# rainerzufalldererste/hypersonic-rANS

Hardware: AMD Instinct MI355X
Metric: decode MiB/s (bit-exact) on 100 MB stream (higher is better)
Workload: dtype u32 state / u16 word / u8 symbol (integer)

## Files before the change

hypersonic_rans_amd/csrc/kernels_common.h:

```cpp
#ifndef HSRANS_KERNELS_COMMON_H
#define HSRANS_KERNELS_COMMON_H

namespace hsrans
{


typedef uint32_t u32x4 __attribute__((ext_vector_type(4)));

constexpr uint32_t kRingSlots = 4;
constexpr uint32_t kChunkBytes = 512;
constexpr uint32_t kRingBytes = kRingSlots * kChunkBytes;
constexpr uint32_t kWaveRingBytes = kRingBytes + 256;
constexpr uint32_t kFastRingBytes = kRingBytes + kChunkBytes;
constexpr uint32_t kConsume = 1u << 15;
#ifndef HSRANS_HAVE_STAMPS
#define HSRANS_HAVE_STAMPS 0
#endif
#define HSRANS_STAMPS(kp) (HSRANS_HAVE_STAMPS && (kp).stamps != nullptr)
constexpr uint32_t kSingleMirror = 256;

constexpr int kModePack = 0;
constexpr int kModePackM1 = 1;
constexpr int kModeTwoLevel = 2;
constexpr int kModePack64 = 3;

constexpr int kModeRank = 4;
constexpr int kModeSpill = 5;

__host__ __device__ constexpr uint32_t table_bytes_for(int mode, uint32_t bits)
{
  return mode == kModeSpill ? 0u
         : mode == kModeTwoLevel ? (1u << bits) + 1024
         : mode == kModePack64 ? 8u << bits
         : mode == kModeRank ? (1u << bits) + 2048u
                               : 4u << bits;
}

__host__ __device__ constexpr bool fast_ring_mode(int mode) { return mode == kModePack64 || mode == kModeRank; }
__host__ __device__ constexpr bool table_first_mode(int mode) { return mode == kModeRank; }

__device__ __forceinline__ uint32_t lds_address(const void *p)
{
  return (uint32_t)(uintptr_t)(const __attribute__((address_space(3))) uint8_t *)p;
}
__device__ __forceinline__ uint32_t uni(uint32_t v) { return __builtin_amdgcn_readfirstlane(v); }
__device__ __forceinline__ uint64_t uni64(uint64_t v)
{
  return (uint64_t)uni((uint32_t)v) | ((uint64_t)uni((uint32_t)(v >> 32)) << 32);
}

#ifndef HSRANS_STORE_POLICY
#define HSRANS_STORE_POLICY " nt"
#endif
#ifndef HSRANS_STORE_POLICY_DIRECT
#define HSRANS_STORE_POLICY_DIRECT " sc0 sc1"
#endif
#define HSRANS_STORE_U32(ptr, v) asm volatile("global_store_dword %0, %1, off" HSRANS_STORE_POLICY : : "v"(ptr), "v"(v) : "memory")
#define HSRANS_STORE_U32_SADDR(base, voff, v) asm volatile("global_store_dword %0, %1, %2" HSRANS_STORE_POLICY : : "v"(voff), "v"(v), "s"(base) : "memory")
template <bool WT>
__device__ __forceinline__ void store_u32(uint8_t *ptr, uint32_t v)
{
  if (WT)
    asm volatile("global_store_dword %0, %1, off" HSRANS_STORE_POLICY_DIRECT : : "v"(ptr), "v"(v) : "memory");
  else
    asm volatile("global_store_dword %0, %1, off" HSRANS_STORE_POLICY : : "v"(ptr), "v"(v) : "memory");
}
template <bool WT>
__device__ __forceinline__ void store_u32_saddr(uint8_t *base, uint32_t voff, uint32_t v)
{
  if (WT)
    asm volatile("global_store_dword %0, %1, %2" HSRANS_STORE_POLICY_DIRECT : : "v"(voff), "v"(v), "s"(base) : "memory");
  else
    asm volatile("global_store_dword %0, %1, %2" HSRANS_STORE_POLICY : : "v"(voff), "v"(v), "s"(base) : "memory");
}

template <bool WT>
__device__ __forceinline__ void store_u8(uint8_t *ptr, uint32_t v)
{
  if (WT)
    asm volatile("global_store_byte %0, %1, off sc0 sc1" : : "v"(ptr), "v"(v) : "memory");
  else
    *ptr = (uint8_t)v;
}
template <bool WT>
__device__ __forceinline__ void store_u128(u32x4 *ptr, u32x4 v)
{
  if (WT)
    asm volatile("global_store_dwordx4 %0, %1, off sc0 sc1" : : "v"(ptr), "v"(v) : "memory");
  else
    *ptr = v;
}

__device__ __forceinline__ uint64_t groups_of(uint32_t S, uint64_t bytes) { return S == 64 ? bytes >> 6 : S == 32 ? bytes >> 5 : bytes / S; }
struct Recip
{
  uint32_t d, inv;
};
__host__ __device__ __forceinline__ Recip recip_of(uint32_t d)
{
  Recip r;
  r.d = d ? d : 1;
  r.inv = 0xFFFFFFFFu / r.d;
  return r;
}
__device__ __forceinline__ uint32_t share_of(uint32_t a, uint32_t n, const Recip &r)
{
  const uint64_t wide = (uint64_t)a * n;
  if (wide >> 32)
    return (uint32_t)(wide / r.d);
  const uint32_t v = (uint32_t)wide;
  uint32_t q = __umulhi(v, r.inv);
  if (v - q * r.d >= r.d)
    q++;
  return q;
}

#define HSRANS_HIST_IN_RANGE(c, off) ((off) >= (c).stream_lo && (off) <= (c).stream_len && (c).stream_len - (off) >= 512)

__device__ __forceinline__ uint32_t lane_to_byte(uint32_t j) { return (j & 0x23u) | ((j & 0x04u) << 2) | ((j & 0x18u) >> 1); }

struct WaveCtx
{
  const uint8_t *stream;
  uint64_t stream_len;
  uint64_t stream_lo;
  uint8_t *out;
  uint64_t out_cap;
  uint32_t *status;
  uint32_t bits, S, lane;
  uint32_t v_mask, v_bits;
  uint8_t *rings;
  uint8_t *table;
  uint8_t *table_b;
  const uint2 *gtable;
  uint16_t *scratch_cnt;
  uint16_t *scratch_cum;
};

#define HSRANS_STREAM_LOAD_FLAGS ""
struct StreamWin
{
  u32x4 rs;
  uint64_t base;
};

struct Ring
{
  uint32_t voff0;
  uint32_t k;
  uint32_t cur;
  uint32_t lds;
  uint32_t clog;
  uint32_t mirror_lanes;
  uint32_t vm, seq1, seq2, seq3;
  uint32_t st1, st2;
#if HSRANS_HAVE_STAMPS
  uint32_t diag_wait = 0, diag_store = 0;
#endif
};

__device__ __forceinline__ void ring_bind(Ring &r, const uint8_t *lds_ring, uint32_t clog = 9, bool whole_chunk_mirror = false)
{
  r.lds = uni(lds_address(lds_ring));
  r.clog = clog;
  r.mirror_lanes = whole_chunk_mirror ? (clog == 9 ? 0xFFFFFFFFu : 0xFFFFu) : clog == 9 ? 0xFFu : 0xFu;
}
__device__ __forceinline__ uint32_t ring_bytes(const Ring &r) { return kRingSlots << r.clog; }

__device__ __forceinline__ void ring_request(const StreamWin &sw, const Ring &r, const WaveCtx &c, uint32_t chunk, bool with_mirror = true)
{
  const uint32_t voff = r.voff0 + (chunk << r.clog) + c.lane * 16;
  const uint32_t slot = chunk & (kRingSlots - 1);
  const uint32_t dst = uni(r.lds + (slot << r.clog));
  const uint32_t lanes = r.clog == 9 ? 0xFFFFFFFFu : 0xFFFFu;
  asm volatile("s_nop 4\n\ts_mov_b32 m0, %1\n\ts_mov_b64 exec, %3\n\tbuffer_load_dwordx4 %0, %2, 0 offen" HSRANS_STREAM_LOAD_FLAGS " lds\n\ts_mov_b64 exec, -1"
               :
               : "v"(voff), "s"(dst), "s"(sw.rs), "s"((uint64_t)lanes)
               : "memory");
  if (slot == 0 && with_mirror)
    asm volatile("s_mov_b32 m0, %1\n\ts_mov_b64 exec, %3\n\tbuffer_load_dwordx4 %0, %2, 0 offen" HSRANS_STREAM_LOAD_FLAGS " lds\n\ts_mov_b64 exec, -1"
                 :
                 : "v"(voff), "s"(uni(r.lds + ring_bytes(r))), "s"(sw.rs), "s"((uint64_t)r.mirror_lanes)
                 : "memory");
}

__device__ __forceinline__ void ring_request_mirror0(const StreamWin &sw, const Ring &r, const WaveCtx &c)
{
  const uint32_t voff = r.voff0 + c.lane * 16;
  asm volatile("s_nop 4\n\ts_mov_b32 m0, %1\n\ts_mov_b64 exec, %3\n\tbuffer_load_dwordx4 %0, %2, 0 offen" HSRANS_STREAM_LOAD_FLAGS " lds\n\ts_mov_b64 exec, -1"
               :
               : "v"(voff), "s"(uni(r.lds + ring_bytes(r))), "s"(sw.rs), "s"((uint64_t)r.mirror_lanes)
               : "memory");
}

__device__ __forceinline__ void win_open(StreamWin &sw, const WaveCtx &c, uint64_t pos, uint64_t limit)
{
  pos = uni64(pos);
  limit = uni64(limit);
  if (limit > c.stream_len)
    limit = c.stream_len;
  const uint64_t a0 = pos & ~(uint64_t)15;
  const uint64_t left = a0 < limit && a0 >= c.stream_lo ? (limit - a0 + 15) & ~(uint64_t)15 : 0;
  const uint64_t addr = (uint64_t)(uintptr_t)c.stream + a0;
  sw.rs.x = uni((uint32_t)addr);
  sw.rs.y = uni((uint32_t)(addr >> 32) & 0xFFFF);
  sw.rs.z = uni((uint32_t)(left > 0xFFFFFFFFull ? 0xFFFFFFFFull : left));
  sw.rs.w = 0x00020000;
  sw.base = a0;
}

#ifndef HSRANS_RING_AHEAD
#define HSRANS_RING_AHEAD 3
#endif
static_assert(HSRANS_RING_AHEAD == 2 || HSRANS_RING_AHEAD == 3, "the ring has 4 slots: the cursor's chunk + 2 or 3 requested ones");

__device__ __forceinline__ void ring_begin(const StreamWin &sw, Ring &r, const WaveCtx &c, uint64_t pos, bool issue = true, bool later = false)
{
  pos = uni64(pos);
  const uint32_t rel = (uint32_t)(pos - sw.base);
  r.voff0 = rel & ~15u;
  r.cur = (rel - r.voff0) >> 1;
  r.k = 0;
  r.st1 = r.st2 = 0;
  r.vm = 0;
  if (issue)
  {
    ring_request(sw, r, c, 0, !later);
    ring_request(sw, r, c, 1);
  }
  r.vm += 3;
  r.seq1 = r.vm;
  if (issue && !later)
    ring_request(sw, r, c, 2);
  r.seq2 = ++r.vm;
  if (HSRANS_RING_AHEAD == 3)
  {
    if (issue && !later)
      ring_request(sw, r, c, 3);
    r.vm++;
  }
  r.seq3 = r.vm;
}
__device__ __forceinline__ void ring_begin_rest(const StreamWin &sw, Ring &r, const WaveCtx &c)
{
  ring_request_mirror0(sw, r, c);
  ring_request(sw, r, c, 2);
  if (HSRANS_RING_AHEAD == 3)
    ring_request(sw, r, c, 3);
}

__device__ __forceinline__ void ring_ready()
{
  if (HSRANS_RING_AHEAD == 3)
    asm volatile("s_waitcnt vmcnt(2)" ::: "memory");
  else
    asm volatile("s_waitcnt vmcnt(1)" ::: "memory");
}
__device__ __forceinline__ void ring_ready(uint32_t &x)
{
  if (HSRANS_RING_AHEAD == 3)
    asm volatile("s_waitcnt vmcnt(2)" : "+v"(x)::"memory");
  else
    asm volatile("s_waitcnt vmcnt(1)" : "+v"(x)::"memory");
}
__device__ __forceinline__ void ring_ready(uint32_t &xa, uint32_t &xb)
{
  if (HSRANS_RING_AHEAD == 3)
    asm volatile("s_waitcnt vmcnt(2)" : "+v"(xa), "+v"(xb)::"memory");
  else
    asm volatile("s_waitcnt vmcnt(1)" : "+v"(xa), "+v"(xb)::"memory");
}

__device__ __forceinline__ void ring_init(StreamWin &sw, Ring &r, const WaveCtx &c, uint64_t pos, uint32_t &x)
{
  win_open(sw, c, pos, c.stream_len);
  ring_begin(sw, r, c, pos);
  ring_ready(x);
}

__device__ __forceinline__ void ring_advance(const StreamWin &sw, Ring &r, const WaveCtx &c)
{
  if ((r.cur >> (r.clog - 1)) > r.k)
  {
    r.k++;
    ring_request(sw, r, c, r.k + HSRANS_RING_AHEAD);
    r.vm += ((r.k + HSRANS_RING_AHEAD) & (kRingSlots - 1)) == 0 ? 2 : 1;
    r.seq1 = r.seq2;
    r.seq2 = r.seq3;
    r.seq3 = r.vm;
    if (HSRANS_RING_AHEAD == 2)
      r.seq2 = r.vm;
    asm volatile("s_waitcnt vmcnt(2)" ::: "memory");
  }
}

__device__ __forceinline__ void wait_vm_at_most(uint32_t n)
{
  if (n >= 8)
    asm volatile("s_waitcnt vmcnt(8)" ::: "memory");
  else if (n >= 6)
    asm volatile("s_waitcnt vmcnt(6)" ::: "memory");
  else if (n >= 4)
    asm volatile("s_waitcnt vmcnt(4)" ::: "memory");
  else if (n >= 2)
    asm volatile("s_waitcnt vmcnt(2)" ::: "memory");
  else if (n == 1)
    asm volatile("s_waitcnt vmcnt(1)" ::: "memory");
  else
    asm volatile("s_waitcnt vmcnt(0)" ::: "memory");
}

__device__ __forceinline__ void ring_advance_exact(const StreamWin &sw, Ring &r, const WaveCtx &c)
{
  if ((r.cur >> (r.clog - 1)) > r.k)
  {
    r.k++;
    ring_request(sw, r, c, r.k + HSRANS_RING_AHEAD);
    r.vm += ((r.k + HSRANS_RING_AHEAD) & (kRingSlots - 1)) == 0 ? 2 : 1;
    r.seq1 = r.seq2;
    r.seq2 = r.seq3;
    r.seq3 = r.vm;
    if (HSRANS_RING_AHEAD == 2)
      r.seq2 = r.vm;
    wait_vm_at_most(r.vm - r.seq1);
  }
}

__device__ __forceinline__ uint64_t ring_pos(const StreamWin &sw, const Ring &r) { return sw.base + r.voff0 + (uint64_t)r.cur * 2; }

__host__ __device__ constexpr bool pack64_marks(uint32_t total, uint32_t nthreads)
{
  return (nthreads & (nthreads - 1)) == 0 && nthreads >= 64 && total >= 1024 && total / (nthreads < total / 4 ? nthreads : total / 4) <= 8;
}
template <int CTRL, int ROW_MASK>
__device__ __forceinline__ uint32_t max_dpp(uint32_t v)
{
  const uint32_t o = (uint32_t)__builtin_amdgcn_update_dpp(0, (int)v, CTRL, ROW_MASK, 0xF, true);
  return v > o ? v : o;
}
__device__ __forceinline__ uint32_t wave_scan_max(uint32_t v)
{
  v = max_dpp<0x111, 0xF>(v);
  v = max_dpp<0x112, 0xF>(v);
  v = max_dpp<0x114, 0xF>(v);
  v = max_dpp<0x118, 0xF>(v);
  v = max_dpp<0x142, 0xA>(v);
  v = max_dpp<0x143, 0xC>(v);
  return v;
}
__device__ __forceinline__ void pack64_zero_marks(uint2 *tab, uint32_t total, uint32_t tid, uint32_t nthreads)
{
  for (uint32_t q = tid; q < total / 4; q += nthreads)
    ((uint32_t *)tab)[q] = 0;
}
__device__ __forceinline__ void pack64_mark4(uint2 *tab, uint32_t total, uint32_t s0, uint32_t excl, uint32_t c0, uint32_t c1, uint32_t c2, uint32_t c3)
{
  uint8_t *mk = (uint8_t *)tab;
  const uint32_t u0 = excl, u1 = u0 + c0, u2 = u1 + c1, u3 = u2 + c2;
  if (c0 != 0 && u0 < total)
    mk[u0] = (uint8_t)s0;
  if (c1 != 0 && u1 < total)
    mk[u1] = (uint8_t)(s0 + 1);
  if (c2 != 0 && u2 < total)
    mk[u2] = (uint8_t)(s0 + 2);
  if (c3 != 0 && u3 < total)
    mk[u3] = (uint8_t)(s0 + 3);
}
template <typename SYNC>
__device__ __forceinline__ void pack64_from_marks(uint2 *tab, const uint16_t *cnt, const uint16_t *cum, uint32_t total, uint32_t tid, uint32_t nthreads, SYNC sync)
{
  const uint32_t active = nthreads < total / 4 ? nthreads : total / 4;
  const uint32_t per = total / active;
  const bool mine = tid < active;
  uint32_t w0 = 0, w1 = 0, prev = 0;
  if (mine)
  {
    const uint32_t lane = tid & 63;
    const uint32_t first = (tid - lane) * per;
    uint32_t before = 0;
#pragma unroll
    for (uint32_t k = 0; k < 4; k++)
      before += (uint32_t)__builtin_popcountll(__ballot((uint32_t)cum[64 * k + lane] <= first));
    const uint32_t *mk = (const uint32_t *)tab + tid * (per / 4);
    w0 = mk[0];
    w1 = per == 8 ? mk[1] : 0;
    uint32_t top = 0;
#pragma unroll
    for (uint32_t j = 0; j < 8; j++)
    {
      const uint32_t b = ((j < 4 ? w0 : w1) >> (8 * (j & 3))) & 0xFF;
      top = b > top ? b : top;
    }
    const uint32_t incl = wave_scan_max(top);
    prev = (uint32_t)__builtin_amdgcn_update_dpp(0, (int)incl, 0x138, 0xF, 0xF, true);
    const uint32_t base = before - 1;
    prev = prev > base ? prev : base;
  }
  sync();
  if (mine)
  {
    const uint32_t slot0 = tid * per;
    uint32_t s = prev;
#pragma unroll
    for (uint32_t j = 0; j < 8; j++)
      if (j < per)
      {
        const uint32_t b = ((j < 4 ? w0 : w1) >> (8 * (j & 3))) & 0xFF;
        s = b > s ? b : s;
        tab[slot0 + j] = make_uint2((uint32_t)cnt[s] | (s << 24), slot0 + j - (uint32_t)cum[s]);
      }
  }
}

template <int MODE, bool BLOCK_SYNC, bool MARKS = true>
__device__ bool build_table(const WaveCtx &c, uint64_t hist_off, uint32_t tid, uint32_t nthreads)
{
  auto sync = [&]() {
    if (BLOCK_SYNC)
      __syncthreads();
    else
    {
      __builtin_amdgcn_fence(__ATOMIC_RELEASE, "wavefront");
      __builtin_amdgcn_wave_barrier();
      __builtin_amdgcn_fence(__ATOMIC_ACQUIRE, "wavefront");
    }
  };
  if (MODE == kModeSpill)
  {
    if (tid == 0)
      atomicOr(c.status, kStatusBadHist);
    return false;
  }
  uint16_t *cnt = c.scratch_cnt;
  uint16_t *cum = c.scratch_cum;
  const uint32_t total = 1u << c.bits;
  bool good = true;

  if (!BLOCK_SYNC)
    asm volatile("s_waitcnt vmcnt(0)" ::: "memory");
  sync();
  const bool in_range = HSRANS_HIST_IN_RANGE(c, hist_off);
  const bool marks = MARKS && MODE == kModePack64 && BLOCK_SYNC && pack64_marks(total, nthreads);
  for (uint32_t s = tid; s < 256; s += nthreads)
    cnt[s] = in_range ? *(const uint16_t *)(c.stream + hist_off + 2 * s) : (uint16_t)0;
  if (marks)
    pack64_zero_marks((uint2 *)c.table, total, tid, nthreads);
  sync();
  if (tid < 64)
  {
    const uint32_t c0 = cnt[4 * tid], c1 = cnt[4 * tid + 1], c2 = cnt[4 * tid + 2], c3 = cnt[4 * tid + 3];
    const uint32_t mine = c0 + c1 + c2 + c3;
    uint32_t incl = mine;
#pragma unroll
    for (int d = 1; d < 64; d <<= 1)
    {
      const uint32_t up = __shfl_up(incl, d, 64);
      if (tid >= (uint32_t)d)
        incl += up;
    }
    const uint32_t excl = incl - mine;
    cum[4 * tid] = (uint16_t)excl;
    cum[4 * tid + 1] = (uint16_t)(excl + c0);
    cum[4 * tid + 2] = (uint16_t)(excl + c0 + c1);
    cum[4 * tid + 3] = (uint16_t)(excl + c0 + c1 + c2);
    if (marks)
      pack64_mark4((uint2 *)c.table, total, 4 * tid, excl, c0, c1, c2, c3);
    good = (uint32_t)__shfl(incl, 63, 64) == total;
    if (!good && tid == 0)
      atomicOr(c.status, kStatusBadHist);
  }
  sync();
  if (!BLOCK_SYNC && !good)
    return false;

  if (MODE == kModePack64 && marks)
    pack64_from_marks((uint2 *)c.table, cnt, cum, total, tid, nthreads, sync);
// ... 157 lines not shown
__device__ __forceinline__ void run_groups_impl(uint32_t &x, const StreamWin &sw, Ring &r, const WaveCtx &c, uint64_t &o_ref, uint32_t steps)
{
  uint64_t o = uni64(o_ref);
  const uint32_t S = FULL ? 64 : c.S;
  const bool act = FULL || c.lane < S;
  const unsigned long long act_mask = FULL ? ~0ull : __builtin_amdgcn_ballot_w64(act);
  constexpr uint32_t kSymByte = (MODE == kModePack64 || MODE == kModeRank || MODE == kModeSpill) ? 3 : 0;
  const OutLanes ol = out_lanes(c.lane, S);

  for (; steps >= 4; steps -= 4)
  {
    const uint32_t e0 = group_step<MODE, FULL>(x, r, c, act_mask);
    const uint32_t e1 = group_step<MODE, FULL>(x, r, c, act_mask);
    const uint32_t e2 = group_step<MODE, FULL>(x, r, c, act_mask);
    const uint32_t e3 = group_step<MODE, FULL>(x, r, c, act_mask);
    const uint32_t acc = pack4<kSymByte>(e0, e1, e2, e3, ol);
    uint8_t *row_base = c.out + o;
    if (FULL)
    {
      if (ALLWT)
        store_u32_saddr<true>((uint8_t *)uni64((uint64_t)(uintptr_t)row_base), ol.store_off, acc);
      else
        HSRANS_STORE_U32_SADDR((uint8_t *)uni64((uint64_t)(uintptr_t)row_base), ol.store_off, acc);
      r.vm++;
    }
    else if (act)
    {
      if (ALLWT)
        store_u32<true>(row_base + ol.store_off, acc);
      else
        HSRANS_STORE_U32((uint32_t *)(row_base + ol.store_off), acc);
    }
    o += 4 * S;
    if (FULL)
      ring_advance_exact(sw, r, c);
    else
      ring_advance(sw, r, c);
  }
  const uint32_t p = lane_to_byte(c.lane);
  for (; steps > 0; steps--)
  {
    const uint32_t e = group_step<MODE, FULL>(x, r, c, act_mask);
    if (act)
      store_u8<ALLWT>(c.out + o + p, (e >> (8 * kSymByte)) & 0xFFu);
    o += S;
  }
  ring_advance(sw, r, c);
  o_ref = o;
}

#define HSRANS_FAST_GROUP(P0, P1)                                                                                                                    \
  "v_and_b32 %[t], %[x], %[vmask]\n\t"                                                                                                               \
  "v_lshl_add_u32 %[t], %[t], 3, %[stab]\n\t"                                                                                                        \
  "ds_read_b64 v[" #P0 ":" #P1 "], %[t]\n\t"                                                                                                         \
  "v_lshrrev_b32 %[x], %[vbits], %[x]\n\t"                                                                                                           \
  "s_waitcnt lgkmcnt(0)\n\t"                                                                                                                         \
  "v_mad_u32_u24 %[x], v" #P0 ", %[x], v" #P1 "\n\t"                                                                                                 \
  "v_cmpx_gt_u32 vcc, %[lim], %[x]\n\t"                                                                                                              \
  "s_nop 1\n\t"                                                                                                                                      \
  "v_mbcnt_lo_u32_b32 %[t], vcc_lo, 0\n\t"                                                                                                           \
  "v_mbcnt_hi_u32_b32 %[t], vcc_hi, %[t]\n\t"                                                                                                        \
  "v_lshl_add_u32 %[t], %[t], 1, %[sa]\n\t"                                                                                                          \
  "ds_read_u16 %[t], %[t]\n\t"                                                                                                                       \
  "s_bcnt1_i32_b64 %[st], vcc\n\t"                                                                                                                   \
  "s_lshl1_add_u32 %[sa], %[st], %[sa]\n\t"                                                                                                          \
  "s_waitcnt lgkmcnt(0)\n\t"                                                                                                                         \
  "v_lshl_or_b32 %[x], %[x], 16, %[t]\n\t"                                                                                                           \
  "s_mov_b64 exec, -1\n\t"

__device__ __forceinline__ uint32_t fast_groups4(uint32_t &x, uint32_t &s_addr, const WaveCtx &c, uint32_t s_table)
{
  uint32_t acc, t, st;
  asm volatile(HSRANS_FAST_GROUP(52, 53) HSRANS_FAST_GROUP(54, 55) HSRANS_FAST_GROUP(56, 57) HSRANS_FAST_GROUP(58, 59)
               "v_perm_b32 %[acc], v54, v52, %[selp]\n\t"
               "v_perm_b32 %[t], v58, v56, %[selp]\n\t"
               "v_perm_b32 %[acc], %[t], %[acc], %[selq]"
               : [x] "+v"(x), [sa] "+s"(s_addr), [acc] "=&v"(acc), [t] "=&v"(t), [st] "=&s"(st)
               : [vmask] "v"(c.v_mask), [vbits] "v"(c.v_bits), [stab] "s"(s_table), [lim] "s"(kConsume), [selp] "s"(0x0c0c0703u), [selq] "s"(0x05040100u)
               : "v52", "v53", "v54", "v55", "v56", "v57", "v58", "v59", "vcc", "scc", "memory");
  return acc;
}

#define HSRANS_FAST_GROUP_RANK(P0, P1)                                                                                                               \
  "v_and_b32 %[g], %[x], %[vmask]\n\t"                                                                                                               \
  "ds_read_u8 v" #P0 ", %[g] offset:%[off]\n\t"                                                                                                      \
  "v_lshrrev_b32 %[x], %[vbits], %[x]\n\t"                                                                                                           \
  "s_waitcnt lgkmcnt(0)\n\t"                                                                                                                         \
  "v_lshl_add_u32 %[t], v" #P0 ", 3, %[sent]\n\t"                                                                                                    \
  "ds_read_b64 v[" #P0 ":" #P1 "], %[t]\n\t"                                                                                                         \
  "s_waitcnt lgkmcnt(0)\n\t"                                                                                                                         \
  "v_mad_u32_u24 %[x], v" #P0 ", %[x], v" #P1 "\n\t"                                                                                                 \
  "v_add_u32 %[x], %[x], %[g]\n\t"                                                                                                                   \
  "v_cmpx_gt_u32 vcc, %[lim], %[x]\n\t"                                                                                                              \
  "s_nop 1\n\t"                                                                                                                                      \
  "v_mbcnt_lo_u32_b32 %[t], vcc_lo, 0\n\t"                                                                                                           \
  "v_mbcnt_hi_u32_b32 %[t], vcc_hi, %[t]\n\t"                                                                                                        \
  "v_lshl_add_u32 %[t], %[t], 1, %[sa]\n\t"                                                                                                          \
  "ds_read_u16 %[t], %[t]\n\t"                                                                                                                       \
  "s_bcnt1_i32_b64 %[st], vcc\n\t"                                                                                                                   \
  "s_lshl1_add_u32 %[sa], %[st], %[sa]\n\t"                                                                                                          \
  "s_waitcnt lgkmcnt(0)\n\t"                                                                                                                         \
  "v_lshl_or_b32 %[x], %[x], 16, %[t]\n\t"                                                                                                           \
  "s_mov_b64 exec, -1\n\t"

template <uint32_t TABLE_OFF = 0>
__device__ __forceinline__ uint32_t fast_groups4_rank(uint32_t &x, uint32_t &s_addr, const WaveCtx &c, uint32_t s_entries)
{
  uint32_t acc, t, g, st;
  asm volatile(HSRANS_FAST_GROUP_RANK(52, 53) HSRANS_FAST_GROUP_RANK(54, 55) HSRANS_FAST_GROUP_RANK(56, 57) HSRANS_FAST_GROUP_RANK(58, 59)
               "v_perm_b32 %[acc], v54, v52, %[selp]\n\t"
               "v_perm_b32 %[t], v58, v56, %[selp]\n\t"
               "v_perm_b32 %[acc], %[t], %[acc], %[selq]"
               : [x] "+v"(x), [sa] "+s"(s_addr), [acc] "=&v"(acc), [t] "=&v"(t), [g] "=&v"(g), [st] "=&s"(st)
               : [vmask] "v"(c.v_mask), [vbits] "v"(c.v_bits), [sent] "s"(s_entries), [lim] "s"(kConsume), [selp] "s"(0x0c0c0703u), [selq] "s"(0x05040100u),
                 [off] "i"(TABLE_OFF)
               : "v52", "v53", "v54", "v55", "v56", "v57", "v58", "v59", "vcc", "scc", "memory");
  return acc;
}

__device__ __forceinline__ void wait_after_crossing(uint32_t &t1, uint32_t &t2, uint32_t iters, uint32_t k3)
{
  static_assert(HSRANS_RING_AHEAD == 3 || HSRANS_RING_AHEAD == 2, "");
  static_assert(kRingSlots == 4, "");
  uint32_t n, extra;
  asm volatile("s_and_b32 %[extra], %[k3], 3\n\t"
               "s_cmp_lt_u32 %[extra], 2\n\t"
               "s_cselect_b32 %[extra], 3, 2\n\t"
               "s_sub_u32 %[n], %[t2], %[it]\n\t"
               "s_add_u32 %[n], %[n], %[extra]\n\t"
               "s_mov_b32 %[t2], %[t1]\n\t"
               "s_mov_b32 %[t1], %[it]\n\t"
               "s_cmp_ge_u32 %[n], 8\n\t"
               "s_cbranch_scc1 8f\n\t"
               "s_cmp_ge_u32 %[n], 6\n\t"
               "s_cbranch_scc1 6f\n\t"
               "s_cmp_ge_u32 %[n], 4\n\t"
               "s_cbranch_scc1 4f\n\t"
               "s_waitcnt vmcnt(3)\n\t"
               "s_branch 9f\n"
               "4:\n\t"
               "s_waitcnt vmcnt(4)\n\t"
               "s_branch 9f\n"
               "6:\n\t"
               "s_waitcnt vmcnt(6)\n\t"
               "s_branch 9f\n"
               "8:\n\t"
               "s_waitcnt vmcnt(8)\n"
               "9:"
               : [n] "=&s"(n), [extra] "=&s"(extra), [t1] "+s"(t1), [t2] "+s"(t2)
               : [it] "s"(iters), [k3] "s"(k3)
               : "scc", "memory");
}

template <bool STRICT, int MODE = kModePack64, bool WT = false, uint32_t TABLE_OFF = 0>
__device__ __forceinline__ void run_groups_fast(uint32_t &x, const StreamWin &sw, Ring &r, const WaveCtx &c, uint64_t &o_ref, uint32_t &steps)
{
  const OutLanes ol = out_lanes(c.lane, 64);
  const uint32_t s_table = uni(lds_address(c.table));
  uint32_t s_addr = uni(r.lds + ((r.cur << 1) & (kRingBytes - 1)));
  uint32_t next_cross = uni(r.lds + (((r.k + 1) & (kRingSlots - 1)) << 9));
  if (next_cross == r.lds)
    next_cross += kRingBytes;
  uint32_t words0 = r.cur;
  uint32_t moved = 0;
  const uint32_t s_addr0 = s_addr;
  uint8_t *outp = (uint8_t *)uni64((uint64_t)(uintptr_t)(c.out + uni64(o_ref)));
  uint32_t iters = steps >> 2;
  steps &= 3;
  o_ref += (uint64_t)iters * 256;
  uint32_t t1 = iters + r.st1, t2 = iters + r.st2;
  {
    for (; iters != 0; iters--)
    {
      const uint32_t acc = quad_transpose(MODE == kModeRank ? fast_groups4_rank<TABLE_OFF>(x, s_addr, c, TABLE_OFF + (1u << c.bits)) : fast_groups4(x, s_addr, c, s_table), ol.sel_a, ol.sel_b);
#if HSRANS_HAVE_STAMPS && defined(HSRANS_DIAG_STORE_TIME)
      const uint64_t ds0 = __builtin_amdgcn_s_memtime();
      asm volatile("s_waitcnt lgkmcnt(0)" ::: "memory");
#endif
#if !defined(HSRANS_DIAG_NO_STORES)
      store_u32_saddr<WT>((uint8_t *)uni64((uint64_t)(uintptr_t)outp), ol.store_off, acc);
#else
      asm volatile("" ::"v"(acc));
#endif
#if HSRANS_HAVE_STAMPS && defined(HSRANS_DIAG_STORE_TIME)
      r.diag_store += (uint32_t)(__builtin_amdgcn_s_memtime() - ds0);
#endif
      outp += 256;
      if (s_addr >= next_cross)
      {
#if HSRANS_HAVE_STAMPS
        const uint64_t dwt0 = __builtin_amdgcn_s_memtime();
#endif
        r.k++;
        next_cross += kChunkBytes;
        if (s_addr >= r.lds + kRingBytes)
        {
          s_addr -= kRingBytes;
          next_cross -= kRingBytes;
          moved += kRingBytes;
        }
        ring_request(sw, r, c, r.k + HSRANS_RING_AHEAD);
        if (!STRICT && HSRANS_RING_AHEAD == 3)
          wait_after_crossing(t1, t2, iters, r.k + HSRANS_RING_AHEAD);
        else
        {
          if (HSRANS_RING_AHEAD == 3 && r.k <= 2)
            asm volatile("s_waitcnt vmcnt(3)" ::: "memory");
          else if (HSRANS_RING_AHEAD == 3)
            asm volatile("s_waitcnt vmcnt(4)" ::: "memory");
          else
            asm volatile("s_waitcnt vmcnt(2)" ::: "memory");
        }
#if HSRANS_HAVE_STAMPS
        r.diag_wait += (uint32_t)(__builtin_amdgcn_s_memtime() - dwt0);
#endif
      }
    }
  }
  r.cur = words0 + ((s_addr + moved - s_addr0) >> 1);
  r.st1 = t1, r.st2 = t2;
  r.vm = r.seq1 = r.seq2 = r.seq3 = 0;
}

template <int MODE, bool FAST = false, bool STRICT = false, bool WT = false, bool ALLWT = false, uint32_t TABLE_OFF = 0>
__device__ __forceinline__ void run_groups(uint32_t &x, const StreamWin &sw, Ring &r, const WaveCtx &c, uint64_t &o, uint32_t steps)
{
  if (FAST && MODE == kModePack64 && c.S == 64 && r.mirror_lanes == 0xFFFFFFFFu)
    run_groups_fast<STRICT, kModePack64, WT>(x, sw, r, c, o, steps);
  if (FAST && MODE == kModeRank && c.S == 64 && r.mirror_lanes == 0xFFFFFFFFu && uni(lds_address(c.table)) == TABLE_OFF)
    run_groups_fast<STRICT || TABLE_OFF == 0, kModeRank, WT, TABLE_OFF>(x, sw, r, c, o, steps);
  if (c.S == 64)
    run_groups_impl<MODE, true, ALLWT>(x, sw, r, c, o, steps);
  else
    run_groups_impl<MODE, false, ALLWT>(x, sw, r, c, o, steps);
}

template <int MODE>
__device__ __forceinline__ uint32_t group_step_pair(uint32_t &x, Ring &ra, Ring &rb, const WaveCtx &c)
{
  const uint32_t mask = (1u << c.bits) - 1;
  const uint32_t slot = x & c.v_mask;
  const uint32_t q = x >> c.v_bits;
  const uint8_t *tab = c.lane < 32 ? c.table : c.table_b;
  uint32_t e, nx;
  if (MODE == kModePack64)
  {
    const uint2 e2 = ((const uint2 *)tab)[slot];
    e = e2.x;
    nx = __umul24(q, e2.x) + e2.y;
  }
  else if (MODE == kModeSpill)
  {
    const uint2 e2 = c.gtable[slot];
    e = e2.x;
    nx = __umul24(q, e2.x) + e2.y;
  }
  else if (MODE == kModeRank)
  {
    const uint2 e2 = ((const uint2 *)(tab + mask + 1))[tab[slot]];
    e = e2.x;
    nx = __umul24(q, e2.x) + e2.y + slot;
  }
  else if (MODE == kModePack)
  {
    e = ((const uint32_t *)tab)[slot];
    nx = __umul24(q, (e >> 8) & 0xFFF) + (e >> 20);
  }
  else if (MODE == kModePackM1)
  {
    e = ((const uint32_t *)tab)[slot];
    nx = __umul24(q, (e >> 8) & 0xFFF) + q + (e >> 20);
  }
  else
  {
    e = tab[slot];
    const uint32_t fc = ((const uint32_t *)(tab + mask + 1))[e];
    nx = __umul24(q, fc & 0xFFFF) + slot - (fc >> 16);
  }
  const bool low = nx < kConsume;
  const unsigned long long m = __builtin_amdgcn_ballot_w64(low);
  const uint32_t m_lo = (uint32_t)m, m_hi = (uint32_t)(m >> 32);
  const uint32_t rank = __builtin_amdgcn_mbcnt_hi(m_hi, __builtin_amdgcn_mbcnt_lo(m_lo, 0));
  const uint32_t cnt_a = (uint32_t)__popc(m_lo), cnt_b = (uint32_t)__popc(m_hi);
  const uint32_t base_a = ra.lds + ((ra.cur << 1) & (ring_bytes(ra) - 1));
  const uint32_t base_b = rb.lds + ((rb.cur << 1) & (ring_bytes(rb) - 1)) - 2 * cnt_a;
  uint32_t va, vb;
  asm("v_mov_b32 %0, %1" : "=v"(va) : "s"(base_a));
  asm("v_mov_b32 %0, %1" : "=v"(vb) : "s"(base_b));
  const uint32_t vbase = (uint32_t)__builtin_amdgcn_update_dpp((int)va, (int)vb, 0xE4, 0xC, 0xF, false);
  uint32_t waddr;
  asm("v_lshl_add_u32 %0, %1, 1, %2" : "=v"(waddr) : "v"(rank), "v"(vbase));
  uint32_t w = *(const __attribute__((address_space(3))) uint16_t *)(uintptr_t)waddr;
  x = nx;
  asm volatile("s_mov_b64 exec, %2\n\tv_lshl_or_b32 %0, %0, 16, %1\n\ts_mov_b64 exec, -1" : "+v"(x) : "v"(w), "s"(m));
  ra.cur += cnt_a;
  rb.cur += cnt_b;
  return e;
}

struct FastCursor
{
  uint32_t addr, next_cross, addr0, words0, moved;
};
__device__ __forceinline__ FastCursor fast_cursor_open(const Ring &r)
{
  FastCursor f;
  f.addr = uni(r.lds + ((r.cur << 1) & (ring_bytes(r) - 1)));
  f.next_cross = uni(r.lds + (((r.k + 1) & (kRingSlots - 1)) << r.clog));
  if (f.next_cross == r.lds)
    f.next_cross += ring_bytes(r);
  f.addr0 = f.addr;
  f.words0 = r.cur;
  f.moved = 0;
  return f;
}
__device__ __forceinline__ void fast_cursor_cross(FastCursor &f, Ring &r)
{
  r.k++;
  f.next_cross += 1u << r.clog;
  if (f.addr >= r.lds + ring_bytes(r))
  {
    f.addr -= ring_bytes(r);
    f.next_cross -= ring_bytes(r);
    f.moved += ring_bytes(r);
  }
}
__device__ __forceinline__ void fast_cursor_close(const FastCursor &f, Ring &r) { r.cur = f.words0 + ((f.addr + f.moved - f.addr0) >> 1); }

template <int MODE>
__device__ __forceinline__ void pair_bind(Ring &ra, Ring &rb, const WaveCtx &c)
{
  ring_bind(ra, c.rings, 8, fast_ring_mode(MODE));
  ring_bind(rb, c.rings + (fast_ring_mode(MODE) ? 1280 : 1152), 8, fast_ring_mode(MODE));
}

#define HSRANS_PAIR_ADDR                                                                                                                             \
  "v_mbcnt_lo_u32_b32 %[t], vcc_lo, 0\n\t"                                                                                                           \
  "v_mbcnt_hi_u32_b32 %[w], vcc_hi, 0\n\t"                                                                                                           \
  "v_lshl_add_u32 %[t], %[t], 1, %[sa]\n\t"                                                                                                          \
  "v_lshl_add_u32 %[w], %[w], 1, %[sb]\n\t"                                                                                                          \
  "v_cndmask_b32 %[w], %[t], %[w], %[up]\n\t"
#define HSRANS_PAIR_GROUP(P0, P1)                                                                                                                    \
  "v_and_b32 %[t], %[x], %[vmask]\n\t"                                                                                                               \
  "v_lshl_add_u32 %[t], %[t], 3, %[stab]\n\t"                                                                                                        \
  "ds_read_b64 v[" #P0 ":" #P1 "], %[t]\n\t"                                                                                                         \
  "v_lshrrev_b32 %[x], %[vbits], %[x]\n\t"                                                                                                           \
  "s_waitcnt lgkmcnt(0)\n\t"                                                                                                                         \
  "v_mad_u32_u24 %[x], v" #P0 ", %[x], v" #P1 "\n\t"                                                                                                 \
  "v_cmpx_gt_u32 vcc, %[lim], %[x]\n\t"                                                                                                              \
  "s_nop 1\n\t"                                                                                                                                      \
  HSRANS_PAIR_ADDR                                                                                                                                   \
  "ds_read_u16 %[w], %[w]\n\t"                                                                                                                       \
  "s_bcnt1_i32_b32 %[st], vcc_lo\n\t"                                                                                                                \
  "s_lshl1_add_u32 %[sa], %[st], %[sa]\n\t"                                                                                                          \
  "s_bcnt1_i32_b32 %[st], vcc_hi\n\t"                                                                                                                \
  "s_lshl1_add_u32 %[sb], %[st], %[sb]\n\t"                                                                                                          \
  "s_waitcnt lgkmcnt(0)\n\t"                                                                                                                         \
  "v_lshl_or_b32 %[x], %[x], 16, %[w]\n\t"                                                                                                           \
  "s_mov_b64 exec, -1\n\t"

__device__ __forceinline__ uint32_t pair_groups4(uint32_t &x, uint32_t &s_a, uint32_t &s_b, const WaveCtx &c, uint32_t s_table)
{
  uint32_t acc, t, w, st;
  asm volatile(HSRANS_PAIR_GROUP(52, 53) HSRANS_PAIR_GROUP(54, 55) HSRANS_PAIR_GROUP(56, 57) HSRANS_PAIR_GROUP(58, 59)
               "v_perm_b32 %[acc], v54, v52, %[selp]\n\t"
               "v_perm_b32 %[t], v58, v56, %[selp]\n\t"
               "v_perm_b32 %[acc], %[t], %[acc], %[selq]"
               : [x] "+v"(x), [sa] "+s"(s_a), [sb] "+s"(s_b), [acc] "=&v"(acc), [t] "=&v"(t), [w] "=&v"(w), [st] "=&s"(st)
               : [vmask] "v"(c.v_mask), [vbits] "v"(c.v_bits), [stab] "s"(s_table), [lim] "s"(kConsume), [selp] "s"(0x0c0c0703u), [selq] "s"(0x05040100u),
                 [up] "s"(0xFFFFFFFF00000000ull)
               : "v52", "v53", "v54", "v55", "v56", "v57", "v58", "v59", "vcc", "scc", "memory");
  return acc;
}

#define HSRANS_PAIR_GROUP_RANK(P0, P1)                                                                                                               \
  "v_and_b32 %[g], %[x], %[vmask]\n\t"                                                                                                               \
  "ds_read_u8 v" #P0 ", %[g]\n\t"                                                                                                                    \
  "v_lshrrev_b32 %[x], %[vbits], %[x]\n\t"                                                                                                           \
  "s_waitcnt lgkmcnt(0)\n\t"                                                                                                                         \
  "v_lshl_add_u32 %[t], v" #P0 ", 3, %[sent]\n\t"                                                                                                    \
  "ds_read_b64 v[" #P0 ":" #P1 "], %[t]\n\t"                                                                                                         \
  "s_waitcnt lgkmcnt(0)\n\t"                                                                                                                         \
  "v_mad_u32_u24 %[x], v" #P0 ", %[x], v" #P1 "\n\t"                                                                                                 \
// ... 228 lines not shown
```

hypersonic_rans_amd/csrc/kernels_direct.h:

```cpp
#ifndef HSRANS_KERNELS_DIRECT_H
#define HSRANS_KERNELS_DIRECT_H

namespace hsrans
{

typedef const __attribute__((address_space(4))) uint64_t *kptr64;
typedef const __attribute__((address_space(4))) uint32_t *kptr32;

struct DirectPiece
{
  uint64_t words, out, limit;
  uint32_t steps, tail;
};

__device__ __forceinline__ DirectPiece direct_piece(const WaveCtx &c, const PersistentArgs &pa, uint32_t ch)
{
  const kptr64 p = (kptr64)(uintptr_t)(pa.pieces + ch);
  DirectPiece d;
  d.words = p[0];
  d.out = p[1];
  const uint32_t st = ((kptr32)p)[8];
  const uint32_t tf = ((kptr32)p)[9];
  d.steps = st;
  d.tail = tf & 0xFFFFu;
  d.limit = ch + 1 < pa.n_chains ? p[6] : c.stream_len;
  return d;
}

template <int MODE>
__device__ __forceinline__ void run_direct_span(const WaveCtx &c, const KParams &kp, uint32_t waves, uint32_t w, uint32_t ch, uint32_t end, bool check_hist)
{
  const PersistentArgs &pa = kp.pa;
  const uint32_t W = gridDim.x * waves;
  const uint64_t t_entry = HSRANS_STAMPS(kp) ? __builtin_amdgcn_s_memrealtime() : 0;
  const uint64_t c_entry = HSRANS_STAMPS(kp) ? __builtin_amdgcn_s_memtime() : 0;
  uint64_t t_table = 0, t_ready = 0, t_static = 0;
#if HSRANS_HAVE_STAMPS
  uint32_t diag_wait = 0, diag_store = 0;
#endif
  const bool host_table = (MODE == kModePack64 || MODE == kModeRank || MODE == kModeSpill) && pa.table != nullptr;
  if (kp.finish != nullptr && w == 0 && c.lane == 0)
    kp.finish[W] = __builtin_amdgcn_s_memrealtime();
  if (!host_table)
    build_table<MODE, true>(c, pa.hist_off, threadIdx.x, blockDim.x);
  auto fetch_table = [&]() {
    if (MODE != kModeSpill)
    {
      const uint32_t entries = table_bytes_for(MODE, c.bits) / 8;
      for (uint32_t i = threadIdx.x * 2; i < entries; i += blockDim.x * 2)
        *(u32x4 *)(c.table + (uint64_t)i * 8) = *(const u32x4 *)(pa.table + i);
    }
    if (check_hist && threadIdx.x < 64)
    {
      bool same = HSRANS_HIST_IN_RANGE(c, pa.hist_off) || pa.hist_off + 512 <= c.stream_lo;
      if (same && pa.hist_off >= c.stream_lo)
      {
        const uint64_t mine = *(const uint64_t *)(pa.hist_copy + 4 * c.lane);
        uint64_t theirs = 0;
        for (int b = 3; b >= 0; b--)
          theirs = (theirs << 16) | *(const uint16_t *)(c.stream + pa.hist_off + 8 * c.lane + 2 * b);
        same = mine == theirs;
      }
      if (__builtin_amdgcn_ballot_w64(!same) != 0 && c.lane == 0)
        atomicOr(c.status, kStatusBadHist);
    }
    if (MODE != kModeSpill)
      __syncthreads();
    if (HSRANS_STAMPS(kp))
      t_table = __builtin_amdgcn_s_memrealtime();
  };
  const uint32_t n = pa.n_chains;
  if (ch < n)
  {
    StreamWin sw;
    Ring r;
    ring_bind(r, c.rings, 9, fast_ring_mode(MODE) && c.S == 64);
    uint32_t x = c.lane < c.S ? pa.states[(uint64_t)ch * c.S + c.lane] : 0;
    const DirectPiece d = direct_piece(c, pa, ch);
    const kptr64 plast = (kptr64)(uintptr_t)(pa.pieces + (end - 1));
    const uint64_t run_limit = end < n ? plast[6] : c.stream_len;
    const uint32_t last_steps = ((kptr32)plast)[8], last_tail = ((kptr32)plast)[9] & 0xFFFFu;
    const uint64_t run_end_out = plast[1] + (uint64_t)last_steps * c.S;
    win_open(sw, c, d.words, run_limit);
#if !defined(HSRANS_PROLOGUE_SPLIT) || HSRANS_PROLOGUE_SPLIT
    ring_begin(sw, r, c, d.words, true, true);
    if (host_table)
      fetch_table();
    ring_begin_rest(sw, r, c);
    asm volatile("s_waitcnt vmcnt(3)" : "+v"(x)::"memory");
#else
    ring_begin(sw, r, c, d.words);
    if (host_table)
      fetch_table();
    ring_ready(x);
#endif
    if (HSRANS_STAMPS(kp))
      t_ready = __builtin_amdgcn_s_memrealtime();
    uint64_t o = d.out;
    run_groups<MODE, true, false, true>(x, sw, r, c, o, (uint32_t)groups_of(c.S, run_end_out - o));
    run_tail<MODE>(x, r, c, o, end == n ? last_tail : 0);
#if HSRANS_HAVE_STAMPS
    diag_wait += r.diag_wait, diag_store += r.diag_store;
#endif
  }
  else if (host_table)
    fetch_table();
  if (HSRANS_STAMPS(kp))
    t_static = __builtin_amdgcn_s_memrealtime();
  if (kp.finish != nullptr && c.lane == 0)
    kp.finish[w] = __builtin_amdgcn_s_memrealtime();
  if (HSRANS_STAMPS(kp) && c.lane == 0)
  {
    uint64_t *st = kp.stamps + (uint64_t)w * 8;
    st[0] = t_entry;
    st[1] = t_table;
    st[2] = t_ready;
    st[3] = __builtin_amdgcn_s_memrealtime();
    st[4] = t_static;
    st[5] = __builtin_amdgcn_s_memtime() - c_entry;
    uint32_t hw_id, xcc_id;
    asm volatile("s_getreg_b32 %0, hwreg(HW_REG_HW_ID)\n\ts_getreg_b32 %1, hwreg(HW_REG_XCC_ID)" : "=s"(hw_id), "=s"(xcc_id));
    st[6] = (uint64_t)hw_id | ((uint64_t)xcc_id << 32);
#if HSRANS_HAVE_STAMPS
    st[7] = (uint64_t)diag_wait | ((uint64_t)diag_store << 32);
#endif
  }
}

template <int MODE>
__device__ void run_direct(const WaveCtx &c, const KParams &kp, uint32_t waves, uint32_t w)
{
  const uint32_t n = kp.pa.n_chains;
  const uint32_t R = kp.pa.run_chains ? kp.pa.run_chains : 1;
  const uint32_t ch = w * R;
  run_direct_span<MODE>(c, kp, waves, w, ch, ch + R < n ? ch + R : n, blockIdx.x == 0);
}

template <int MODE>
__device__ void run_direct_pair(const WaveCtx &c, const KParams &kp, uint32_t waves, uint32_t w)
{
  const PersistentArgs &pa = kp.pa;
  const uint32_t W = gridDim.x * waves;
  const uint64_t t_entry = HSRANS_STAMPS(kp) ? __builtin_amdgcn_s_memrealtime() : 0;
  uint64_t t_ready = 0, t_static = 0;
  StreamWin sw;
  Ring ra, rb;
  pair_bind<MODE>(ra, rb, c);
  const bool host_table = (MODE == kModePack64 || MODE == kModeRank || MODE == kModeSpill) && pa.table != nullptr;
  if (!host_table)
    build_table<MODE, true>(c, pa.hist_off, threadIdx.x, blockDim.x);
  bool table_pending = host_table && MODE != kModeSpill;
  if (host_table && blockIdx.x == 0 && threadIdx.x < 64)
  {
    bool same = HSRANS_HIST_IN_RANGE(c, pa.hist_off) || pa.hist_off + 512 <= c.stream_lo;
    if (same && pa.hist_off >= c.stream_lo)
    {
      const uint64_t mine = *(const uint64_t *)(pa.hist_copy + 4 * c.lane);
      uint64_t theirs = 0;
      for (int b = 3; b >= 0; b--)
        theirs = (theirs << 16) | *(const uint16_t *)(c.stream + pa.hist_off + 8 * c.lane + 2 * b);
      same = mine == theirs;
    }
    if (__builtin_amdgcn_ballot_w64(!same) != 0 && c.lane == 0)
      atomicOr(c.status, kStatusBadHist);
  }
  auto copy_table = [&]() {
    const uint32_t entries = table_bytes_for(MODE, c.bits) / 8;
    for (uint32_t i = threadIdx.x * 2; i < entries; i += blockDim.x * 2)
      *(u32x4 *)(c.table + (uint64_t)i * 8) = *(const u32x4 *)(pa.table + i);
    __syncthreads();
  };
  uint32_t a = 2 * w, end = pa.n_chains;
  bool have = a < pa.n_chains;
  while (true)
  {
    if (have)
    {
      const bool have_b = a + 1 < end;
      const DirectPiece da = direct_piece(c, pa, a);
      const DirectPiece db = have_b ? direct_piece(c, pa, a + 1) : da;
      win_open(sw, c, da.words, have_b ? db.limit : da.limit);
      ring_begin(sw, ra, c, da.words, true, true);
      if (have_b)
        ring_begin(sw, rb, c, db.words, true, true);
      uint32_t x = pa.states[(uint64_t)((c.lane < 32 || !have_b) ? a : a + 1) * 32 + (c.lane & 31)];
      if (table_pending)
      {
        copy_table();
        table_pending = false;
      }
      ring_begin_rest(sw, ra, c);
      if (have_b)
        ring_begin_rest(sw, rb, c);
      if (have_b)
        asm volatile("s_waitcnt vmcnt(6)" : "+v"(x)::"memory");
      else
        asm volatile("s_waitcnt vmcnt(3)" : "+v"(x)::"memory");
      if (HSRANS_STAMPS(kp) && t_ready == 0)
        t_ready = __builtin_amdgcn_s_memrealtime();
      uint64_t oa = da.out, ob = db.out;
      uint32_t sa = da.steps, sb = have_b ? db.steps : 0;
      const uint32_t both = have_b ? (sa < sb ? sa : sb) & ~3u : 0;
      run_pair_groups<MODE, true, true>(x, sw, ra, rb, c, oa, ob, both);
      sa -= both;
      sb -= both;
      uint32_t xb = __shfl(x, (c.lane & 31) + 32, 64);
      run_groups<MODE>(xb, sw, rb, c, ob, sb);
      run_tail<MODE>(xb, rb, c, ob, have_b ? db.tail : 0);
      run_groups<MODE>(x, sw, ra, c, oa, sa);
      run_tail<MODE>(x, ra, c, oa, da.tail);
    }
    if (HSRANS_STAMPS(kp) && t_static == 0)
      t_static = __builtin_amdgcn_s_memrealtime();
    a += 2 * W;
    have = a < pa.n_chains;
    if (!have)
      break;
  }
  if (table_pending)
    copy_table();
  if (HSRANS_STAMPS(kp) && c.lane == 0)
  {
    uint64_t *st = kp.stamps + (uint64_t)w * 8;
    st[0] = t_entry;
    st[1] = t_ready;
    st[2] = t_ready;
    st[3] = __builtin_amdgcn_s_memrealtime();
    st[4] = t_static;
    st[5] = 0;
    st[6] = 0;
  }
}

template <int MODE>
__global__ void __launch_bounds__(1024) __attribute__((amdgpu_num_sgpr(80))) k_decode_direct(KParams kp)
{
  extern __shared__ u32x4 smem_v[];
  uint8_t *smem = (uint8_t *)smem_v;
  const uint32_t waves = blockDim.x >> 6;
  const uint32_t wave = uni(threadIdx.x >> 6);
  WaveCtx c;
  c.stream = kp.stream;
  c.stream_len = kp.stream_len;
  c.stream_lo = kp.stream_lo;
  c.out = kp.out;
  c.out_cap = kp.out_cap;
  c.status = kp.status;
  c.bits = kp.pa.bits;
  c.S = kp.pa.S;
  c.lane = threadIdx.x & 63;
  asm volatile("v_mov_b32 %0, %1" : "=v"(c.v_mask) : "s"((1u << c.bits) - 1));
  asm volatile("v_mov_b32 %0, %1" : "=v"(c.v_bits) : "s"(c.bits));
// ... 47 lines not shown
```

Before: 2.453 million.

## Ramp up ring prefetch: issue two chunks at start, request owed chunks lazily

Measured after the change: 2.452 million. Within noise of the previous version (-0.0%).

```diff
diff --git a/hypersonic_rans_amd/csrc/kernels_common.h b/hypersonic_rans_amd/csrc/kernels_common.h
--- a/hypersonic_rans_amd/csrc/kernels_common.h
+++ b/hypersonic_rans_amd/csrc/kernels_common.h
@@ -154,6 +154,7 @@
   uint32_t mirror_lanes;
   uint32_t vm, seq1, seq2, seq3;
   uint32_t st1, st2;
+  uint32_t lag = 0;
 #if HSRANS_HAVE_STAMPS
   uint32_t diag_wait = 0, diag_store = 0;
 #endif
@@ -213,8 +214,11 @@
 #define HSRANS_RING_AHEAD 3
 #endif
 static_assert(HSRANS_RING_AHEAD == 2 || HSRANS_RING_AHEAD == 3, "the ring has 4 slots: the cursor's chunk + 2 or 3 requested ones");
-
-__device__ __forceinline__ void ring_begin(const StreamWin &sw, Ring &r, const WaveCtx &c, uint64_t pos, bool issue = true, bool later = false)
+#ifndef HSRANS_PROLOGUE_SPLIT
+#define HSRANS_PROLOGUE_SPLIT 2
+#endif
+
+__device__ __forceinline__ void ring_begin(const StreamWin &sw, Ring &r, const WaveCtx &c, uint64_t pos, bool issue = true, bool later = false, bool ramp = false)
 {
   pos = uni64(pos);
   const uint32_t rel = (uint32_t)(pos - sw.base);
@@ -222,7 +226,16 @@
   r.cur = (rel - r.voff0) >> 1;
   r.k = 0;
   r.st1 = r.st2 = 0;
+  r.lag = 0;
   r.vm = 0;
+  if (ramp)
+  {
+    ring_request(sw, r, c, 0, false);
+    ring_request(sw, r, c, 1);
+    r.vm = r.seq1 = r.seq2 = r.seq3 = 2;
+    r.lag = HSRANS_RING_AHEAD - 1;
+    return;
+  }
   if (issue)
   {
     ring_request(sw, r, c, 0, !later);
@@ -278,13 +291,25 @@
   ring_ready(x);
 }
 
+__device__ __forceinline__ uint32_t ring_request_owed(const StreamWin &sw, Ring &r, const WaveCtx &c, uint32_t upto)
+{
+  uint32_t ops = 0;
+  for (uint32_t chunk = upto - r.lag; chunk <= upto; chunk++)
+  {
+    ring_request(sw, r, c, chunk);
+    ops += (chunk & (kRingSlots - 1)) == 0 ? 2 : 1;
+  }
+  r.lag = 0;
+  return ops;
+}
+
 __device__ __forceinline__ void ring_advance(const StreamWin &sw, Ring &r, const WaveCtx &c)
 {
   if ((r.cur >> (r.clog - 1)) > r.k)
   {
     r.k++;
-    ring_request(sw, r, c, r.k + HSRANS_RING_AHEAD);
-    r.vm += ((r.k + HSRANS_RING_AHEAD) & (kRingSlots - 1)) == 0 ? 2 : 1;
+    const uint32_t ops = ring_request_owed(sw, r, c, r.k + HSRANS_RING_AHEAD);
+    r.vm += ops;
     r.seq1 = r.seq2;
     r.seq2 = r.seq3;
     r.seq3 = r.vm;
@@ -315,13 +340,15 @@
   if ((r.cur >> (r.clog - 1)) > r.k)
   {
     r.k++;
-    ring_request(sw, r, c, r.k + HSRANS_RING_AHEAD);
-    r.vm += ((r.k + HSRANS_RING_AHEAD) & (kRingSlots - 1)) == 0 ? 2 : 1;
+    const bool owed = r.lag != 0;
+    r.vm += ring_request_owed(sw, r, c, r.k + HSRANS_RING_AHEAD);
     r.seq1 = r.seq2;
     r.seq2 = r.seq3;
     r.seq3 = r.vm;
     if (HSRANS_RING_AHEAD == 2)
       r.seq2 = r.vm;
+    if (owed)
+      r.seq1 = r.seq2 = r.seq3 = r.vm;
     wait_vm_at_most(r.vm - r.seq1);
   }
 }
@@ -785,7 +812,7 @@
                : "scc", "memory");
 }
 
-template <bool STRICT, int MODE = kModePack64, bool WT = false, uint32_t TABLE_OFF = 0>
+template <bool STRICT, int MODE = kModePack64, bool WT = false, uint32_t TABLE_OFF = 0, bool RAMP = false>
 __device__ __forceinline__ void run_groups_fast(uint32_t &x, const StreamWin &sw, Ring &r, const WaveCtx &c, uint64_t &o_ref, uint32_t &steps)
 {
   const OutLanes ol = out_lanes(c.lane, 64);
@@ -802,23 +829,59 @@
   steps &= 3;
   o_ref += (uint64_t)iters * 256;
   uint32_t t1 = iters + r.st1, t2 = iters + r.st2;
-  {
-    for (; iters != 0; iters--)
-    {
-      const uint32_t acc = quad_transpose(MODE == kModeRank ? fast_groups4_rank<TABLE_OFF>(x, s_addr, c, TABLE_OFF + (1u << c.bits)) : fast_groups4(x, s_addr, c, s_table), ol.sel_a, ol.sel_b);
+  auto four_groups = [&]() {
+    const uint32_t acc = quad_transpose(MODE == kModeRank ? fast_groups4_rank<TABLE_OFF>(x, s_addr, c, TABLE_OFF + (1u << c.bits)) : fast_groups4(x, s_addr, c, s_table), ol.sel_a, ol.sel_b);
 #if HSRANS_HAVE_STAMPS && defined(HSRANS_DIAG_STORE_TIME)
-      const uint64_t ds0 = __builtin_amdgcn_s_memtime();
-      asm volatile("s_waitcnt lgkmcnt(0)" ::: "memory");
+    const uint64_t ds0 = __builtin_amdgcn_s_memtime();
+    asm volatile("s_waitcnt lgkmcnt(0)" ::: "memory");
 #endif
 #if !defined(HSRANS_DIAG_NO_STORES)
-      store_u32_saddr<WT>((uint8_t *)uni64((uint64_t)(uintptr_t)outp), ol.store_off, acc);
+    store_u32_saddr<WT>((uint8_t *)uni64((uint64_t)(uintptr_t)outp), ol.store_off, acc);
 #else
-      asm volatile("" ::"v"(acc));
+    asm volatile("" ::"v"(acc));
 #endif
 #if HSRANS_HAVE_STAMPS && defined(HSRANS_DIAG_STORE_TIME)
-      r.diag_store += (uint32_t)(__builtin_amdgcn_s_memtime() - ds0);
+    r.diag_store += (uint32_t)(__builtin_amdgcn_s_memtime() - ds0);
 #endif
-      outp += 256;
+    outp += 256;
+  };
+  if (RAMP && r.lag != 0 && iters != 0)
+  {
+    four_groups();
+    iters--;
+    r.lag--;
+    ring_request(sw, r, c, r.k + HSRANS_RING_AHEAD - r.lag);
+    const uint32_t tp = iters;
+    while (iters != 0 && s_addr < next_cross)
+    {
+      four_groups();
+      iters--;
+    }
+    if (s_addr >= next_cross)
+    {
+#if HSRANS_HAVE_STAMPS
+      const uint64_t dwt0 = __builtin_amdgcn_s_memtime();
+#endif
+      r.k++;
+      next_cross += kChunkBytes;
+      if (s_addr >= r.lds + kRingBytes)
+      {
+        s_addr -= kRingBytes;
+        next_cross -= kRingBytes;
+        moved += kRingBytes;
+      }
+      const uint32_t ops = ring_request_owed(sw, r, c, r.k + HSRANS_RING_AHEAD);
+      wait_vm_at_most(tp - iters + ops);
+      t1 = t2 = iters;
+#if HSRANS_HAVE_STAMPS
+      r.diag_wait += (uint32_t)(__builtin_amdgcn_s_memtime() - dwt0);
+#endif
+    }
+  }
+  {
+    for (; iters != 0; iters--)
+    {
+      four_groups();
       if (s_addr >= next_cross)
       {
 #if HSRANS_HAVE_STAMPS
@@ -855,13 +918,13 @@
   r.vm = r.seq1 = r.seq2 = r.seq3 = 0;
 }
 
-template <int MODE, bool FAST = false, bool STRICT = false, bool WT = false, bool ALLWT = false, uint32_t TABLE_OFF = 0>
+template <int MODE, bool FAST = false, bool STRICT = false, bool WT = false, bool ALLWT = false, uint32_t TABLE_OFF = 0, bool RAMP = false>
 __device__ __forceinline__ void run_groups(uint32_t &x, const StreamWin &sw, Ring &r, const WaveCtx &c, uint64_t &o, uint32_t steps)
 {
   if (FAST && MODE == kModePack64 && c.S == 64 && r.mirror_lanes == 0xFFFFFFFFu)
-    run_groups_fast<STRICT, kModePack64, WT>(x, sw, r, c, o, steps);
+    run_groups_fast<STRICT, kModePack64, WT, 0, RAMP>(x, sw, r, c, o, steps);
   if (FAST && MODE == kModeRank && c.S == 64 && r.mirror_lanes == 0xFFFFFFFFu && uni(lds_address(c.table)) == TABLE_OFF)
-    run_groups_fast<STRICT || TABLE_OFF == 0, kModeRank, WT, TABLE_OFF>(x, sw, r, c, o, steps);
+    run_groups_fast<STRICT || TABLE_OFF == 0, kModeRank, WT, TABLE_OFF, RAMP>(x, sw, r, c, o, steps);
   if (c.S == 64)
     run_groups_impl<MODE, true, ALLWT>(x, sw, r, c, o, steps);
   else
diff --git a/hypersonic_rans_amd/csrc/kernels_direct.h b/hypersonic_rans_amd/csrc/kernels_direct.h
--- a/hypersonic_rans_amd/csrc/kernels_direct.h
+++ b/hypersonic_rans_amd/csrc/kernels_direct.h
@@ -82,7 +82,12 @@
     const uint32_t last_steps = ((kptr32)plast)[8], last_tail = ((kptr32)plast)[9] & 0xFFFFu;
     const uint64_t run_end_out = plast[1] + (uint64_t)last_steps * c.S;
     win_open(sw, c, d.words, run_limit);
-#if !defined(HSRANS_PROLOGUE_SPLIT) || HSRANS_PROLOGUE_SPLIT
+#if HSRANS_PROLOGUE_SPLIT == 2
+    ring_begin(sw, r, c, d.words, true, false, true);
+    if (host_table)
+      fetch_table();
+    asm volatile("s_waitcnt vmcnt(0)" : "+v"(x)::"memory");
+#elif HSRANS_PROLOGUE_SPLIT
     ring_begin(sw, r, c, d.words, true, true);
     if (host_table)
       fetch_table();
@@ -97,7 +102,7 @@
     if (HSRANS_STAMPS(kp))
       t_ready = __builtin_amdgcn_s_memrealtime();
     uint64_t o = d.out;
-    run_groups<MODE, true, false, true>(x, sw, r, c, o, (uint32_t)groups_of(c.S, run_end_out - o));
+    run_groups<MODE, true, false, true, false, 0, HSRANS_PROLOGUE_SPLIT == 2>(x, sw, r, c, o, (uint32_t)groups_of(c.S, run_end_out - o));
     run_tail<MODE>(x, r, c, o, end == n ? last_tail : 0);
 #if HSRANS_HAVE_STAMPS
     diag_wait += r.diag_wait, diag_store += r.diag_store;
```
